# GLAD-RUC/DistEGNN

Measured on NVIDIA H100. Metric: graph_steps_per_sec, higher is better.
Workload: dtype f32

## Files before the change

distegnn_b200/csrc/edge_layer_cs.cu:

```cuda
#include <cuda_fp16.h>
#include <string.h>

#include "common.cuh"
#include "det.cuh"
#include "tc16.cuh"
#include "tile_mma.cuh"

namespace degnn {

struct EdgeCsArgs {
    int64_t N, E;
    const int32_t* E_dev;
    int A;
    unsigned flags;
    const int32_t* row;
    const int32_t* col;
    const float* ea;
    const float* x4;
    const float* P;
    const float* Q;
    const float* w1r;
    const float* w1e;
    const float* w2;
    const float* b2;
    const float* wc;
    const float* bc;
    const float* w3;
    float* agg_m;
    float* agg_x;
    float* slots;
};

constexpr int CS_WG = 4;
constexpr int CS_THREADS = 128 * CS_WG, CS_WARPS = CS_THREADS / 32;
constexpr int CS_TILE = 64;
constexpr int CS_QROW = 72;
constexpr int CS_WBUF = 16 * CS_QROW;
constexpr int CS_IDX = 64;
constexpr int CS_W = 64 * 64;
constexpr int CS_SMEM_BYTES = 4 * CS_W * 2
                              + CS_WARPS * 2 * 8
                              + (4 * H + DISTEGNN_MAX_EDGE_ATTR * H) * 4
                              + CS_WARPS * 2 * CS_WBUF * 4
                              + CS_WARPS * CS_IDX * 4
                              + CS_WARPS * 16 * 8 * 4;
constexpr uint32_t CS_LBO = 1024;

template <int AT, bool LASTL, bool DET>
__global__ void __launch_bounds__(CS_THREADS, 1) edge_layer_cs_kernel(const EdgeCsArgs a) {
    using namespace tmma;
    constexpr int AMAX = AT >= 0 ? (AT > 0 ? AT : 1) : DISTEGNN_MAX_EDGE_ATTR;
    constexpr int AR = (AT == 1 || AT == 2) ? AT : 0;
    constexpr bool need_m = !LASTL;
    __half* W2hi = reinterpret_cast<__half*>(degnn_dyn_smem);
    __half* W2lo = W2hi + CS_W;
    __half* Wchi = W2lo + CS_W;
    __half* Wclo = Wchi + CS_W;
    uint64_t* bars = reinterpret_cast<uint64_t*>(Wclo + CS_W);
    float* b2s = reinterpret_cast<float*>(bars + CS_WARPS * 2);
    float* bcs = b2s + H;
    float* w3s = bcs + H;
    float* w1rs = w3s + H;
    float* w1es = w1rs + H;
    float* qbufs = w1es + DISTEGNN_MAX_EDGE_ATTR * H;
    int* idx_all = reinterpret_cast<int*>(qbufs + CS_WARPS * 2 * CS_WBUF);
    float* xs_all = reinterpret_cast<float*>(idx_all + CS_WARPS * CS_IDX);

    const int tid = threadIdx.x;
    const int lane = tid & 31;
    const int warp = tid >> 5;
    const int wg = warp >> 2;
    const int w = warp & 3;
    const int g = lane >> 2, q = lane & 3;
    const int A = AT >= 0 ? AT : a.A;
    const bool normalize = a.flags & DISTEGNN_FLAG_NORMALIZE;

    tc16::stage_weight<CS_THREADS>(W2hi, W2lo, a.w2, 0, 64, tid, SILU_T_IN);
    tc16::stage_weight<CS_THREADS>(Wchi, Wclo, a.wc, 0, 64, tid);
    if (tid < H) {
        b2s[tid] = a.b2[tid] * SILU_T_IN;
        bcs[tid] = a.bc[tid] * SILU_T_IN;
        w3s[tid] = a.w3[tid] * SILU_T_OUT;
        w1rs[tid] = a.w1r[tid];
    }
    for (int i = tid; i < DISTEGNN_MAX_EDGE_ATTR * H; i += CS_THREADS) w1es[i] = i < A * H ? a.w1e[i] : 0.f;
    for (int i = tid; i < CS_WARPS * 2 * CS_WBUF / 4; i += CS_THREADS)
        reinterpret_cast<float4*>(qbufs)[i] = make_float4(0.f, 0.f, 0.f, 0.f);
    if (tid == 0) {
        for (int i = 0; i < CS_WARPS * 2; ++i) mbar_init(&bars[i], 1);
        fence_mbar_init();
    }
    fence_proxy_async_smem();
    __syncthreads();

    float* qb = qbufs + warp * 2 * CS_WBUF;
    int* nidx = idx_all + warp * CS_IDX;
    float* xs = xs_all + warp * 16 * 8 + 8 * (lane & 15);
    uint64_t* qbar = bars + 2 * warp;
    const uint64_t bW2hi = make_desc(smem_u32(W2hi), CS_LBO, 128), bW2lo = make_desc(smem_u32(W2lo), CS_LBO, 128);
    const uint64_t bWchi = make_desc(smem_u32(Wchi), CS_LBO, 128), bWclo = make_desc(smem_u32(Wclo), CS_LBO, 128);

    const int64_t nE = a.E_dev ? min((int64_t)__ldg(a.E_dev), a.E) : a.E;
    const int64_t num_tiles = (nE + CS_TILE - 1) / CS_TILE;
    const int64_t stride = (int64_t)gridDim.x * CS_WG;
    int64_t tile = (int64_t)blockIdx.x * CS_WG + wg;

    auto edge_of = [&](int64_t tl) { return tl * CS_TILE + 16 * w + lane; };
    auto has_edge = [&](int64_t tl) { return lane < 16 && tl < num_tiles && edge_of(tl) < nE; };
    auto fetch_q = [&](int64_t tl, int b, int col_e, bool v) {
        if (lane == 0) {
            const int64_t nv = min((int64_t)16, max((int64_t)0, nE - (tl * CS_TILE + 16 * w)));
            mbar_expect_tx(qbar + b, (uint32_t)nv * (H * 4));
        }
        if (v) bulk_g2s(qb + b * CS_WBUF + lane * CS_QROW, a.Q + (size_t)col_e * H, H * 4, qbar + b);
    };

    int row_c = -1;
    float dx = 0.f, dy = 0.f, dz = 0.f, radial = 0.f;
    auto set_geometry = [&](float4 xi, float4 xj) {
        dx = xi.x - xj.x; dy = xi.y - xj.y; dz = xi.z - xj.z;
        radial = dx * dx + dy * dy + dz * dz;
        if (normalize) {
            const float inv = 1.0f / (sqrtf(radial) + 1e-8f);
            dx *= inv; dy *= inv; dz *= inv;
        }
    };
    float ea_c[AR > 0 ? AR : 1], n_ea[AR > 0 ? AR : 1];
#pragma unroll
    for (int k = 0; k < (AR > 0 ? AR : 1); ++k) ea_c[k] = n_ea[k] = 0.f;
    int n_row = -1, n_col = 0;

    if (tile < num_tiles) {
        int col_c = 0;
        if (has_edge(tile)) {
            const int64_t e = edge_of(tile);
            row_c = __ldg(a.row + e);
            col_c = __ldg(a.col + e);
#pragma unroll
            for (int k = 0; k < AR; ++k) ea_c[k] = __ldg(a.ea + e * AR + k);
        }
        fetch_q(tile, 0, col_c, row_c >= 0);
        set_geometry(ldg4(a.x4 + (size_t)max(row_c, 0) * 4), ldg4(a.x4 + (size_t)col_c * 4));
        if (has_edge(tile + stride)) {
            const int64_t e = edge_of(tile + stride);
            n_row = __ldg(a.row + e);
            n_col = __ldg(a.col + e);
#pragma unroll
            for (int k = 0; k < AR; ++k) n_ea[k] = __ldg(a.ea + e * AR + k);
        }
    }

    for (int it = 0; tile < num_tiles; ++it, tile += stride) {
        const int64_t ntile = tile + stride, nntile = ntile + stride;
        const int b = it & 1;
        float* qcur = qb + b * CS_WBUF;

        int cont_row = -1;
        if constexpr (DET) {
            const int64_t e0 = tile * CS_TILE + 16 * w;
            const int r0 = __shfl_sync(FULL, row_c, 0);
            if (r0 >= 0 && e0 > 0 && __ldg(a.row + e0 - 1) == r0) cont_row = r0;
        }
        float* const slot = DET ? a.slots + (size_t)(tile * 4 + w) * DET_EDGE_SLOT : nullptr;

        if (ntile < num_tiles) fetch_q(ntile, b ^ 1, n_col, n_row >= 0);
        if (n_row >= 0) {
            cp_async16(xs, a.x4 + (size_t)n_row * 4);
            cp_async16(xs + 4, a.x4 + (size_t)n_col * 4);
            prefetch_l1(a.P + (size_t)n_row * H);
            prefetch_l1(a.P + (size_t)n_row * H + 32);
        }
        if (has_edge(nntile)) {
            const int64_t e = edge_of(nntile);
            cp_async4(nidx + lane, a.row + e);
            cp_async4(nidx + 16 + lane, a.col + e);
            if (AT == 1) cp_async4(nidx + 32 + 2 * lane, a.ea + e);
            if (AT == 2) cp_async8(nidx + 32 + 2 * lane, a.ea + e * 2);
        }
        cp_async_commit();

        const int ra = __shfl_sync(FULL, row_c, g), rb = __shfl_sync(FULL, row_c, g + 8);
        const float rada = __shfl_sync(FULL, radial, g), radb = __shfl_sync(FULL, radial, g + 8);
        float eaa[AMAX], eab[AMAX];
#pragma unroll
        for (int k = 0; k < AMAX; ++k) {
            if (AR > 0) {
                eaa[k] = __shfl_sync(FULL, ea_c[k < AR ? k : 0], g);
                eab[k] = __shfl_sync(FULL, ea_c[k < AR ? k : 0], g + 8);
            } else if (AT < 0) {
                const int64_t e = tile * CS_TILE + 16 * w + g;
                eaa[k] = (k < A && ra >= 0) ? __ldg(a.ea + e * A + k) : 0.f;
                eab[k] = (k < A && rb >= 0) ? __ldg(a.ea + (e + 8) * A + k) : 0.f;
            } else {
                eaa[k] = eab[k] = 0.f;
            }
        }
        const float* pa = a.P + (size_t)max(ra, 0) * H + 2 * q;
        const float* pb = a.P + (size_t)max(rb, 0) * H + 2 * q;
        const float* qa = qcur + g * CS_QROW + 2 * q;
        const float* qbr = qa + 8 * CS_QROW;
        const bool oka = !DET || ra >= 0, okb = !DET || rb >= 0;
        auto pre = [&](int j, const float* prow, const float* qrow, float rad, const float (&ea)[AMAX], bool ok) {
            if (DET && !ok) return bc2(0.f);
            const int c = 8 * j + 2 * q;
            const f32x2 pp = __ldg(reinterpret_cast<const f32x2*>(prow + 8 * j));
            const f32x2 qq = *reinterpret_cast<const f32x2*>(qrow + 8 * j);
            f32x2 p = fma2(bc2(rad), *reinterpret_cast<const f32x2*>(w1rs + c), add2(pp, qq));
#pragma unroll
            for (int k = 0; k < AMAX; ++k)
                if (AT < 0 || k < A)
                    p = fma2(bc2(ea[k]), *reinterpret_cast<const f32x2*>(w1es + k * H + c), p);
            return p;
        };
        uint32_t ahi[16], alo[16];
        float qmax = 0.f;
        auto silu_guard = [&] { return silu_q_overflow(qmax); };
        tc16::RowScales s1;
        mbar_wait(qbar + b, (uint32_t)((it >> 1) & 1));
        tc16::encode_rows<false, true>(
            [&](int j, f32x2& va, f32x2& vb, auto pass) {
                va = pre(j, pa, qa, rada, eaa, oka);
                vb = pre(j, pb, qbr, radb, eab, okb);
                silu4p<decltype(pass)::value != tc16::FAST_PASS>(va, vb, qmax);
            },
            ahi, alo, s1, silu_guard);

        float d[32];
        tc16::mma_f16x3_rA<CS_LBO>(d, ahi, alo, bW2hi, bW2lo);
        const int row_prev = __shfl_up_sync(FULL, row_c, 1);
        const uint32_t M = __ballot_sync(FULL, lane == 0 || row_prev != row_c) & 0xffffu;
        tc16::mma_f16x3_rA_wait(d, ahi, alo);

        qmax = 0.f;
        tc16::RowScales s2;
        tc16::encode_rows<false>(
            [&](int j, f32x2& ma, f32x2& mb, auto pass) {
                const f32x2 bb = *reinterpret_cast<const f32x2*>(b2s + 8 * j + 2 * q);
                ma = fma2(pk2(d[4 * j + 0], d[4 * j + 1]), bc2(s1.inv_a), bb);
                mb = fma2(pk2(d[4 * j + 2], d[4 * j + 3]), bc2(s1.inv_b), bb);
                silu4t<decltype(pass)::value != tc16::FAST_PASS>(ma, mb, qmax);
                if (need_m && decltype(pass)::value != tc16::ENCODE_PASS) {
                    *reinterpret_cast<f32x2*>(qcur + g * CS_QROW + 8 * j + 2 * q) = ma;
                    *reinterpret_cast<f32x2*>(qcur + (g + 8) * CS_QROW + 8 * j + 2 * q) = mb;
                }
            },
            ahi, alo, s2, silu_guard);

        tc16::mma_f16x3_rA<CS_LBO>(d, ahi, alo, bWchi, bWclo);
        if (need_m) {
            __syncwarp();
            const float* colp = qcur + 2 * lane;
            auto flush = [&](f32x2 acc, int e_last) {
                const int rr = __shfl_sync(FULL, row_c, e_last);
                if (rr >= 0) {
                    float v0, v1;
                    upk2(mul2(acc, bc2(SILU_T_OUT)), v0, v1);
                    if constexpr (DET)
                        *reinterpret_cast<float2*>(rr == cont_row ? slot + 2 * lane : a.agg_m + (size_t)rr * H + 2 * lane) =
                            make_float2(v0, v1);
                    else
                        red_add_v2(a.agg_m + (size_t)rr * H + 2 * lane, v0, v1);
                }
            };
            f32x2 s0 = *reinterpret_cast<const f32x2*>(colp);
            if ((M >> 1) == 0u) {
                f32x2 s1 = *reinterpret_cast<const f32x2*>(colp + CS_QROW);
#pragma unroll
                for (int e = 2; e < 16; e += 2) {
                    s0 = add2(s0, *reinterpret_cast<const f32x2*>(colp + e * CS_QROW));
                    s1 = add2(s1, *reinterpret_cast<const f32x2*>(colp + (e + 1) * CS_QROW));
                }
                flush(add2(s0, s1), 15);
            } else {
#pragma unroll
                for (int e = 1; e < 16; ++e) {
                    const f32x2 v = *reinterpret_cast<const f32x2*>(colp + e * CS_QROW);
                    if ((M >> e) & 1u) {
                        flush(s0, e - 1);
                        s0 = v;
                    } else {
                        s0 = add2(s0, v);
                    }
                }
                flush(s0, 15);
            }
        }
        fence_proxy_async_smem();
        __syncwarp();
        tc16::mma_f16x3_rA_wait(d, ahi, alo);

        float phia, phib;
        tc16::phi_head_t(d, s2.inv_a, s2.inv_b, bcs, w3s, q, phia, phib);
        {
            const float fa = __shfl_sync(FULL, phia, 4 * (lane & 7)), fb = __shfl_sync(FULL, phib, 4 * (lane & 7));
            const float phi = (lane & 8) ? fb : fa;
            float sx = dx * phi, sy = dy * phi, sz = dz * phi;
#pragma unroll
            for (int o = 1; o < 16; o <<= 1) {
                const int rk = __shfl_up_sync(FULL, row_c, o);
                const float ox = __shfl_up_sync(FULL, sx, o), oy = __shfl_up_sync(FULL, sy, o), oz = __shfl_up_sync(FULL, sz, o);
                if (lane >= o && rk == row_c) { sx += ox; sy += oy; sz += oz; }
            }
            const int rnext = __shfl_down_sync(FULL, row_c, 1);
            if (row_c >= 0 && (lane == 15 || rnext != row_c)) {
                if constexpr (DET) {
                    float* dst = row_c == cont_row ? slot + H : a.agg_x + (size_t)row_c * 4;
                    dst[0] = sx;
                    dst[1] = sy;
                    dst[2] = sz;
                } else {
                    float* dst = a.agg_x + (size_t)row_c * 4;
                    atomicAdd(dst + 0, sx);
                    atomicAdd(dst + 1, sy);
                    atomicAdd(dst + 2, sz);
                }
            }
        }

        cp_async_wait_all();
        row_c = n_row;
        float4 xi_n = make_float4(0.f, 0.f, 0.f, 0.f), xj_n = xi_n;
        if (n_row >= 0) {
            xi_n = *reinterpret_cast<const float4*>(xs);
            xj_n = *reinterpret_cast<const float4*>(xs + 4);
        }
        set_geometry(xi_n, xj_n);
#pragma unroll
        for (int k = 0; k < AR; ++k) ea_c[k] = n_ea[k];
        n_row = -1;
        if (has_edge(nntile)) {
            n_row = nidx[lane];
            n_col = nidx[16 + lane];
            if (AT == 1) n_ea[0] = __int_as_float(nidx[32 + 2 * lane]);
            if (AT == 2) {
                n_ea[0] = __int_as_float(nidx[32 + 2 * lane]);
                n_ea[AR - 1] = __int_as_float(nidx[33 + 2 * lane]);
            }
        }
    }
}

}

namespace degnn {

template <bool DET>
static int edge_layer_fwd(int64_t n_nodes, int64_t n_edges, int A, int C, int Na, unsigned flags, const int32_t* row,
                          const int32_t* col, const float* edge_attr_sorted, const float* x4, const float* P,
                          const float* Q, const float* layer_params, float* agg_m, float* agg_x,
                          const int32_t* n_edges_dev, void* workspace, int64_t workspace_bytes, void* stream,
                          int max_ctas) {
    if (int rc = check_dims(A, C, Na)) return rc;
    if (n_edges == 0) return DISTEGNN_OK;
    DEGNN_CHECK_ARG(n_nodes > 0 && n_edges > 0, "negative size");
    DEGNN_CHECK_ARG(row && col && x4 && P && Q && layer_params && agg_x, "null pointer");
    DEGNN_CHECK_ARG(A == 0 || edge_attr_sorted, "null edge_attr with edge_attr_nf > 0");
    DEGNN_CHECK_ARG((flags & DISTEGNN_FLAG_LAST) || agg_m, "null agg_m");
    float* slots = nullptr;
    if (DET) {
        if (int rc = det_check_workspace(n_nodes, n_edges, C, workspace, workspace_bytes, "distegnn_edge_layer_fwd_det"))
            return rc;
        slots = det_edge_slots(workspace, n_nodes, C);
    }
    Layout L = make_layout(A, C, Na);
    EdgeCsArgs a;
    a.N = n_nodes; a.E = n_edges; a.E_dev = n_edges_dev; a.A = A; a.flags = flags & 0xffffu;
    a.row = row; a.col = col; a.ea = edge_attr_sorted; a.x4 = x4; a.P = P; a.Q = Q;
    a.w1r = layer_params + L.off[DISTEGNN_P_E_W1R];
    a.w1e = layer_params + L.off[DISTEGNN_P_E_W1E];
    a.w2 = layer_params + L.off[DISTEGNN_P_E_W2];
    a.b2 = layer_params + L.off[DISTEGNN_P_E_B2];
    a.wc = layer_params + L.off[DISTEGNN_P_E_WC];
    a.bc = layer_params + L.off[DISTEGNN_P_E_BC];
    a.w3 = layer_params + L.off[DISTEGNN_P_E_W3];
    a.agg_m = agg_m; a.agg_x = agg_x; a.slots = slots;
    const int64_t tiles = (n_edges + CS_TILE - 1) / CS_TILE;
    int64_t grid = (tiles + CS_WG - 1) / CS_WG;
    if (grid > sm_count()) grid = sm_count();
    if (DET) grid = det_grid(grid, max_ctas);
    auto launch = [&](auto kern) {
        ensure_dynamic_smem((const void*)kern, (int)CS_SMEM_BYTES);
        kern<<<(unsigned)grid, CS_THREADS, CS_SMEM_BYTES, (cudaStream_t)stream>>>(a);
    };
    const bool last = flags & DISTEGNN_FLAG_LAST;
    switch (A) {
        case 0: last ? launch(edge_layer_cs_kernel<0, true, DET>) : launch(edge_layer_cs_kernel<0, false, DET>); break;
        case 1: last ? launch(edge_layer_cs_kernel<1, true, DET>) : launch(edge_layer_cs_kernel<1, false, DET>); break;
        case 2: last ? launch(edge_layer_cs_kernel<2, true, DET>) : launch(edge_layer_cs_kernel<2, false, DET>); break;
        default: last ? launch(edge_layer_cs_kernel<-1, true, DET>) : launch(edge_layer_cs_kernel<-1, false, DET>); break;
    }
    DEGNN_CHECK_LAUNCH();
    return DISTEGNN_OK;
}

int edge_layer_fwd_det(int64_t n_nodes, int64_t n_edges, int A, int C, int Na, unsigned flags, const int32_t* row,
                       const int32_t* col, const float* edge_attr_sorted, const float* x4, const float* P, const float* Q,
                       const float* layer_params, float* agg_m, float* agg_x, const int32_t* n_edges_dev,
                       void* workspace, int64_t workspace_bytes, void* stream, int max_ctas) {
    return edge_layer_fwd<true>(n_nodes, n_edges, A, C, Na, flags, row, col, edge_attr_sorted, x4, P, Q, layer_params,
                                agg_m, agg_x, n_edges_dev, workspace, workspace_bytes, stream, max_ctas);
}

}

extern "C" int distegnn_edge_layer_fwd(int64_t n_nodes, int64_t n_edges, int A, int C, int Na, unsigned flags,
                                       const int32_t* row, const int32_t* col, const float* edge_attr_sorted,
                                       const float* x4, const float* P, const float* Q,
                                       const float* layer_params, float* agg_m, float* agg_x,
                                       const int32_t* n_edges_dev, void* stream) {
    return degnn::edge_layer_fwd<false>(n_nodes, n_edges, A, C, Na, flags, row, col, edge_attr_sorted, x4, P, Q,
                                        layer_params, agg_m, agg_x, n_edges_dev, nullptr, 0, stream, 0);
}

extern "C" int distegnn_edge_layer_fwd_det(int64_t n_nodes, int64_t n_edges, int A, int C, int Na, unsigned flags,
                                           const int32_t* row, const int32_t* col, const float* edge_attr_sorted,
                                           const float* x4, const float* P, const float* Q,
                                           const float* layer_params, float* agg_m, float* agg_x,
                                           const int32_t* n_edges_dev, void* workspace, int64_t workspace_bytes,
                                           void* stream) {
    return degnn::edge_layer_fwd_det(n_nodes, n_edges, A, C, Na, flags, row, col, edge_attr_sorted, x4, P, Q,
                                     layer_params, agg_m, agg_x, n_edges_dev, workspace, workspace_bytes, stream, 0);
}
```

distegnn_b200/csrc/tile_mma.cuh:

```cuda
#pragma once
#include <cuda_runtime.h>
#include <stdint.h>

namespace degnn {

extern __shared__ __align__(1024) uint8_t degnn_dyn_smem[];

namespace tmma {

constexpr uint32_t TM_COLGROUP_BYTES = 2048;
__host__ __device__ constexpr int tm_bytes(int ncols) { return ncols * 128 * 4; }

__device__ __forceinline__ uint32_t smem_u32(const void* p) {
    return (uint32_t)__cvta_generic_to_shared(p);
}

__device__ __forceinline__ uint32_t tm_addr_rc(uint32_t row, uint32_t col) {
    return smem_u32(degnn_dyn_smem) + (col >> 2) * TM_COLGROUP_BYTES + row * 16u + (col & 3u) * 4u;
}
__device__ __forceinline__ uint32_t tm_addr(uint32_t taddr) {
    return tm_addr_rc((taddr >> 16) + (threadIdx.x & 31u), taddr & 0xffffu);
}

__device__ __forceinline__ uint64_t make_desc(uint32_t smem_addr, uint32_t lbo, uint32_t sbo) {
    return (uint64_t)((smem_addr >> 4) & 0x3FFF) | ((uint64_t)((lbo >> 4) & 0x3FFF) << 16) |
           ((uint64_t)((sbo >> 4) & 0x3FFF) << 32);
}

__device__ __forceinline__ void fence_proxy_async_smem() { asm volatile("fence.proxy.async.shared::cta;" ::: "memory"); }

__device__ __forceinline__ void tm_st4(uint32_t taddr, const uint32_t (&r)[4]) {
    asm volatile("st.shared.v4.b32 [%0], {%1,%2,%3,%4};" ::"r"(tm_addr(taddr)), "r"(r[0]), "r"(r[1]), "r"(r[2]), "r"(r[3])
                 : "memory");
}
__device__ __forceinline__ void tm_ld4(uint32_t taddr, uint32_t* r) {
    asm volatile("ld.shared.v4.b32 {%0,%1,%2,%3}, [%4];" : "=r"(r[0]), "=r"(r[1]), "=r"(r[2]), "=r"(r[3]) : "r"(tm_addr(taddr))
                 : "memory");
}
__device__ __forceinline__ void tm_st8(uint32_t taddr, const uint32_t (&r)[8]) {
    tm_st4(taddr, *reinterpret_cast<const uint32_t(*)[4]>(&r[0]));
    tm_st4(taddr + 4, *reinterpret_cast<const uint32_t(*)[4]>(&r[4]));
}
__device__ __forceinline__ void tm_st16(uint32_t taddr, const uint32_t (&r)[16]) {
#pragma unroll
    for (int i = 0; i < 4; ++i) tm_st4(taddr + 4 * i, *reinterpret_cast<const uint32_t(*)[4]>(&r[4 * i]));
}
__device__ __forceinline__ void tm_ld16(uint32_t taddr, uint32_t (&r)[16]) {
#pragma unroll
    for (int i = 0; i < 4; ++i) tm_ld4(taddr + 4 * i, &r[4 * i]);
}
__device__ __forceinline__ void prefetch_l1(const void* p) { asm volatile("prefetch.global.L1 [%0];" ::"l"(p)); }
__device__ __forceinline__ void prefetch_l2(const void* p) { asm volatile("prefetch.global.L2 [%0];" ::"l"(p)); }

__device__ __forceinline__ void wgmma_fence() { asm volatile("wgmma.fence.sync.aligned;" ::: "memory"); }
__device__ __forceinline__ void wgmma_commit() { asm volatile("wgmma.commit_group.sync.aligned;" ::: "memory"); }
__device__ __forceinline__ void wgmma_wait_all() { asm volatile("wgmma.wait_group.sync.aligned 0;" ::: "memory"); }
__device__ __forceinline__ void wgmma_f16_m64n64k16(float (&d)[32], uint64_t a_desc, uint64_t b_desc, uint32_t accumulate) {
    asm volatile(
        "{\n\t"
        ".reg .pred p;\n\t"
        "setp.ne.b32 p, %34, 0;\n\t"
        "wgmma.mma_async.sync.aligned.m64n64k16.f32.f16.f16 "
        "{%0,%1,%2,%3,%4,%5,%6,%7,%8,%9,%10,%11,%12,%13,%14,%15,%16,%17,%18,%19,%20,%21,%22,%23,%24,%25,%26,%27,%28,%29,%30,%31},"
        " %32, %33, p, 1, 1, 0, 0;\n\t"
        "}\n"
        : "+f"(d[0]), "+f"(d[1]), "+f"(d[2]), "+f"(d[3]), "+f"(d[4]), "+f"(d[5]), "+f"(d[6]), "+f"(d[7]), "+f"(d[8]),
          "+f"(d[9]), "+f"(d[10]), "+f"(d[11]), "+f"(d[12]), "+f"(d[13]), "+f"(d[14]), "+f"(d[15]), "+f"(d[16]),
          "+f"(d[17]), "+f"(d[18]), "+f"(d[19]), "+f"(d[20]), "+f"(d[21]), "+f"(d[22]), "+f"(d[23]), "+f"(d[24]),
          "+f"(d[25]), "+f"(d[26]), "+f"(d[27]), "+f"(d[28]), "+f"(d[29]), "+f"(d[30]), "+f"(d[31])
        : "l"(a_desc), "l"(b_desc), "r"(accumulate)
        : "memory");
}
#define DEGNN_WGMMA_RA_D(c)                                                                                             \
    c(d[0]), c(d[1]), c(d[2]), c(d[3]), c(d[4]), c(d[5]), c(d[6]), c(d[7]), c(d[8]), c(d[9]), c(d[10]), c(d[11]),      \
        c(d[12]), c(d[13]), c(d[14]), c(d[15]), c(d[16]), c(d[17]), c(d[18]), c(d[19]), c(d[20]), c(d[21]), c(d[22]),  \
        c(d[23]), c(d[24]), c(d[25]), c(d[26]), c(d[27]), c(d[28]), c(d[29]), c(d[30]), c(d[31])
#define DEGNN_WGMMA_RA_ASM(scale_d)                                                                                     \
    "wgmma.mma_async.sync.aligned.m64n64k16.f32.f16.f16 "                                                               \
    "{%0,%1,%2,%3,%4,%5,%6,%7,%8,%9,%10,%11,%12,%13,%14,%15,%16,%17,%18,%19,%20,%21,%22,%23,%24,%25,%26,%27,%28,%29,%30," \
    "%31}, {%32,%33,%34,%35}, %36, " scale_d ", 1, 1, 0;\n"
template <bool ACCUMULATE>
__device__ __forceinline__ void wgmma_f16_m64n64k16_rA(float (&d)[32], uint32_t a0, uint32_t a1, uint32_t a2, uint32_t a3,
                                                       uint64_t b_desc) {
    if (ACCUMULATE)
        asm volatile(DEGNN_WGMMA_RA_ASM("1") : DEGNN_WGMMA_RA_D("+f")
                     : "r"(a0), "r"(a1), "r"(a2), "r"(a3), "l"(b_desc) : "memory");
    else
        asm volatile(DEGNN_WGMMA_RA_ASM("0") : DEGNN_WGMMA_RA_D("=f")
                     : "r"(a0), "r"(a1), "r"(a2), "r"(a3), "l"(b_desc) : "memory");
}
#undef DEGNN_WGMMA_RA_D
#undef DEGNN_WGMMA_RA_ASM
__device__ __forceinline__ void wgmma_keep(float& r) { asm volatile("" : "+f"(r)::"memory"); }
__device__ __forceinline__ void wgmma_keep(uint32_t& r) { asm volatile("" : "+r"(r)::"memory"); }
__device__ __forceinline__ void frag_rows(int mb, uint32_t& r0, uint32_t& q) {
    const uint32_t w = (threadIdx.x >> 5) & 3u, l = threadIdx.x & 31u;
    r0 = 64u * (uint32_t)mb + 16u * w + (l >> 2);
    q = l & 3u;
}
__device__ __forceinline__ void frag_store(const float (&d)[32], uint32_t col, int mb) {
    uint32_t r0, q;
    frag_rows(mb, r0, q);
#pragma unroll
    for (int j = 0; j < 8; ++j) {
        const uint32_t c = col + 8u * j + 2u * q;
        const uint32_t a0 = tm_addr_rc(r0, c), a1 = tm_addr_rc(r0 + 8u, c);
        asm volatile("st.shared.v2.f32 [%0], {%1,%2};" ::"r"(a0), "f"(d[4 * j]), "f"(d[4 * j + 1]) : "memory");
        asm volatile("st.shared.v2.f32 [%0], {%1,%2};" ::"r"(a1), "f"(d[4 * j + 2]), "f"(d[4 * j + 3]) : "memory");
    }
}
__device__ __forceinline__ void frag_load(float (&d)[32], uint32_t col, int mb) {
    uint32_t r0, q;
    frag_rows(mb, r0, q);
#pragma unroll
    for (int j = 0; j < 8; ++j) {
        const uint32_t c = col + 8u * j + 2u * q;
        asm volatile("ld.shared.v2.f32 {%0,%1}, [%2];" : "=f"(d[4 * j]), "=f"(d[4 * j + 1]) : "r"(tm_addr_rc(r0, c)) : "memory");
        asm volatile("ld.shared.v2.f32 {%0,%1}, [%2];" : "=f"(d[4 * j + 2]), "=f"(d[4 * j + 3]) : "r"(tm_addr_rc(r0 + 8u, c))
                     : "memory");
    }
}

__device__ __forceinline__ void mbar_init(uint64_t* bar, uint32_t count) {
    asm volatile("mbarrier.init.shared::cta.b64 [%0], %1;" ::"r"(smem_u32(bar)), "r"(count) : "memory");
}
__device__ __forceinline__ void fence_mbar_init() { asm volatile("fence.mbarrier_init.release.cluster;" ::: "memory"); }
__device__ __forceinline__ void mbar_expect_tx(uint64_t* bar, uint32_t bytes) {
    asm volatile("mbarrier.arrive.expect_tx.shared::cta.b64 _, [%0], %1;" ::"r"(smem_u32(bar)), "r"(bytes) : "memory");
}
__device__ __forceinline__ void mbar_wait(uint64_t* bar, uint32_t parity) {
    asm volatile(
        "{\n\t"
        ".reg .pred p;\n\t"
        "WAIT_LOOP:\n\t"
        "mbarrier.try_wait.parity.shared::cta.b64 p, [%0], %1;\n\t"
        "@p bra WAIT_DONE;\n\t"
        "bra WAIT_LOOP;\n\t"
        "WAIT_DONE:\n\t"
        "}\n" ::"r"(smem_u32(bar)),
        "r"(parity)
        : "memory");
}

__device__ __forceinline__ void bulk_g2s(void* smem_dst, const void* gsrc, uint32_t bytes, uint64_t* bar) {
    asm volatile("cp.async.bulk.shared::cluster.global.mbarrier::complete_tx::bytes [%0], [%1], %2, [%3];" ::"r"(
                     smem_u32(smem_dst)),
                 "l"(gsrc), "r"(bytes), "r"(smem_u32(bar))
                 : "memory");
}

__device__ __forceinline__ void cp_async16(void* smem_dst, const void* gsrc) {
    asm volatile("cp.async.cg.shared.global [%0], [%1], 16;" ::"r"(smem_u32(smem_dst)), "l"(gsrc) : "memory");
}
__device__ __forceinline__ void cp_async8(void* smem_dst, const void* gsrc) {
    asm volatile("cp.async.ca.shared.global [%0], [%1], 8;" ::"r"(smem_u32(smem_dst)), "l"(gsrc) : "memory");
}
__device__ __forceinline__ void cp_async4(void* smem_dst, const void* gsrc) {
    asm volatile("cp.async.ca.shared.global [%0], [%1], 4;" ::"r"(smem_u32(smem_dst)), "l"(gsrc) : "memory");
}
__device__ __forceinline__ void cp_async_commit() { asm volatile("cp.async.commit_group;" ::: "memory"); }
__device__ __forceinline__ void cp_async_wait_all() { asm volatile("cp.async.wait_group 0;" ::: "memory"); }
__device__ __forceinline__ void red_add_v2(float* gdst, float a, float b) {
    asm volatile("red.global.add.v2.f32 [%0], {%1, %2};" ::"l"(gdst), "f"(a), "f"(b) : "memory");
}

__device__ __forceinline__ void named_bar(uint32_t id, uint32_t nthreads) {
    asm volatile("bar.sync %0, %1;" ::"r"(id), "r"(nthreads) : "memory");
}

}
}
```

Before: 36.47.

## Replace per-row bulk TMA Q gather with warp-cooperative cp.async and 32-bit indexing

Q rows for each tile's column nodes are now gathered with warp-cooperative 16-byte cp.async copies instead of per-lane cp.async.bulk transfers tracked by mbarriers. The mbarrier setup, waits and async-proxy fences are removed, and completion is handled by the existing cp.async wait group plus a syncwarp. Edge, tile and stride indices move from 64-bit to 32-bit arithmetic, with hoisted base pointers, to cut address math. A host check now rejects edge counts near 2^31.

Measured after the change: 37.70 (median of 6 runs). 3.4% higher.

```diff
diff --git a/distegnn_b200/csrc/edge_layer_cs.cu b/distegnn_b200/csrc/edge_layer_cs.cu
--- a/distegnn_b200/csrc/edge_layer_cs.cu
+++ b/distegnn_b200/csrc/edge_layer_cs.cu
@@ -9,7 +9,8 @@
 namespace degnn {
 
 struct EdgeCsArgs {
-    int64_t N, E;
+    int64_t N;
+    int E;
     const int32_t* E_dev;
     int A;
     unsigned flags;
@@ -39,7 +40,6 @@
 constexpr int CS_IDX = 64;
 constexpr int CS_W = 64 * 64;
 constexpr int CS_SMEM_BYTES = 4 * CS_W * 2
-                              + CS_WARPS * 2 * 8
                               + (4 * H + DISTEGNN_MAX_EDGE_ATTR * H) * 4
                               + CS_WARPS * 2 * CS_WBUF * 4
                               + CS_WARPS * CS_IDX * 4
@@ -56,8 +56,7 @@
     __half* W2lo = W2hi + CS_W;
     __half* Wchi = W2lo + CS_W;
     __half* Wclo = Wchi + CS_W;
-    uint64_t* bars = reinterpret_cast<uint64_t*>(Wclo + CS_W);
-    float* b2s = reinterpret_cast<float*>(bars + CS_WARPS * 2);
+    float* b2s = reinterpret_cast<float*>(Wclo + CS_W);
     float* bcs = b2s + H;
     float* w3s = bcs + H;
     float* w1rs = w3s + H;
@@ -86,33 +85,34 @@
     for (int i = tid; i < DISTEGNN_MAX_EDGE_ATTR * H; i += CS_THREADS) w1es[i] = i < A * H ? a.w1e[i] : 0.f;
     for (int i = tid; i < CS_WARPS * 2 * CS_WBUF / 4; i += CS_THREADS)
         reinterpret_cast<float4*>(qbufs)[i] = make_float4(0.f, 0.f, 0.f, 0.f);
-    if (tid == 0) {
-        for (int i = 0; i < CS_WARPS * 2; ++i) mbar_init(&bars[i], 1);
-        fence_mbar_init();
-    }
     fence_proxy_async_smem();
     __syncthreads();
 
     float* qb = qbufs + warp * 2 * CS_WBUF;
     int* nidx = idx_all + warp * CS_IDX;
     float* xs = xs_all + warp * 16 * 8 + 8 * (lane & 15);
-    uint64_t* qbar = bars + 2 * warp;
+    const float* Pq = a.P + 2 * q;
+    asm("" : "+l"(Pq));
     const uint64_t bW2hi = make_desc(smem_u32(W2hi), CS_LBO, 128), bW2lo = make_desc(smem_u32(W2lo), CS_LBO, 128);
     const uint64_t bWchi = make_desc(smem_u32(Wchi), CS_LBO, 128), bWclo = make_desc(smem_u32(Wclo), CS_LBO, 128);
 
-    const int64_t nE = a.E_dev ? min((int64_t)__ldg(a.E_dev), a.E) : a.E;
-    const int64_t num_tiles = (nE + CS_TILE - 1) / CS_TILE;
-    const int64_t stride = (int64_t)gridDim.x * CS_WG;
-    int64_t tile = (int64_t)blockIdx.x * CS_WG + wg;
-
-    auto edge_of = [&](int64_t tl) { return tl * CS_TILE + 16 * w + lane; };
-    auto has_edge = [&](int64_t tl) { return lane < 16 && tl < num_tiles && edge_of(tl) < nE; };
-    auto fetch_q = [&](int64_t tl, int b, int col_e, bool v) {
-        if (lane == 0) {
-            const int64_t nv = min((int64_t)16, max((int64_t)0, nE - (tl * CS_TILE + 16 * w)));
-            mbar_expect_tx(qbar + b, (uint32_t)nv * (H * 4));
-        }
-        if (v) bulk_g2s(qb + b * CS_WBUF + lane * CS_QROW, a.Q + (size_t)col_e * H, H * 4, qbar + b);
+    const int nE = a.E_dev ? min(__ldg(a.E_dev), a.E) : a.E;
+    const int num_tiles = (nE + CS_TILE - 1) / CS_TILE;
+    const int stride = gridDim.x * CS_WG;
+    int tile = blockIdx.x * CS_WG + wg;
+
+    auto edge_of = [&](int tl) { return tl * CS_TILE + 16 * w + lane; };
+    auto has_edge = [&](int tl) { return lane < 16 && tl < num_tiles && edge_of(tl) < nE; };
+    auto fetch_q = [&](int b, int col_e) {
+        const int cols = __shfl_sync(FULL, col_e, (lane & 15) + (lane >> 4));
+        const uint32_t dst = smem_u32(qb + b * CS_WBUF + (lane >> 4) * CS_QROW + 4 * (lane & 15));
+        const char* src = reinterpret_cast<const char*>(a.Q + 4 * (lane & 15));
+        asm("" : "+l"(src));
+#pragma unroll
+        for (int k = 0; k < 8; ++k) {
+            const int c = __shfl_sync(FULL, cols, 2 * k, 16);
+            if (c >= 0) cp_async16(dst + 2 * k * CS_QROW * 4, src + (size_t)(uint32_t)c * (H * 4));
+        }
     };
 
     int row_c = -1;
@@ -133,37 +133,40 @@
     if (tile < num_tiles) {
         int col_c = 0;
         if (has_edge(tile)) {
-            const int64_t e = edge_of(tile);
+            const int e = edge_of(tile);
             row_c = __ldg(a.row + e);
             col_c = __ldg(a.col + e);
 #pragma unroll
-            for (int k = 0; k < AR; ++k) ea_c[k] = __ldg(a.ea + e * AR + k);
-        }
-        fetch_q(tile, 0, col_c, row_c >= 0);
+            for (int k = 0; k < AR; ++k) ea_c[k] = __ldg(a.ea + (size_t)e * AR + k);
+        }
+        fetch_q(0, row_c >= 0 ? col_c : -1);
+        cp_async_commit();
         set_geometry(ldg4(a.x4 + (size_t)max(row_c, 0) * 4), ldg4(a.x4 + (size_t)col_c * 4));
         if (has_edge(tile + stride)) {
-            const int64_t e = edge_of(tile + stride);
+            const int e = edge_of(tile + stride);
             n_row = __ldg(a.row + e);
             n_col = __ldg(a.col + e);
 #pragma unroll
-            for (int k = 0; k < AR; ++k) n_ea[k] = __ldg(a.ea + e * AR + k);
-        }
+            for (int k = 0; k < AR; ++k) n_ea[k] = __ldg(a.ea + (size_t)e * AR + k);
+        }
+        cp_async_wait_all();
+        __syncwarp();
     }
 
     for (int it = 0; tile < num_tiles; ++it, tile += stride) {
-        const int64_t ntile = tile + stride, nntile = ntile + stride;
+        const int nntile = tile + 2 * stride;
         const int b = it & 1;
         float* qcur = qb + b * CS_WBUF;
 
         int cont_row = -1;
         if constexpr (DET) {
-            const int64_t e0 = tile * CS_TILE + 16 * w;
+            const int e0 = tile * CS_TILE + 16 * w;
             const int r0 = __shfl_sync(FULL, row_c, 0);
             if (r0 >= 0 && e0 > 0 && __ldg(a.row + e0 - 1) == r0) cont_row = r0;
         }
         float* const slot = DET ? a.slots + (size_t)(tile * 4 + w) * DET_EDGE_SLOT : nullptr;
 
-        if (ntile < num_tiles) fetch_q(ntile, b ^ 1, n_col, n_row >= 0);
+        fetch_q(b ^ 1, n_row >= 0 ? n_col : -1);
         if (n_row >= 0) {
             cp_async16(xs, a.x4 + (size_t)n_row * 4);
             cp_async16(xs + 4, a.x4 + (size_t)n_col * 4);
@@ -171,11 +174,11 @@
             prefetch_l1(a.P + (size_t)n_row * H + 32);
         }
         if (has_edge(nntile)) {
-            const int64_t e = edge_of(nntile);
+            const int e = edge_of(nntile);
             cp_async4(nidx + lane, a.row + e);
             cp_async4(nidx + 16 + lane, a.col + e);
             if (AT == 1) cp_async4(nidx + 32 + 2 * lane, a.ea + e);
-            if (AT == 2) cp_async8(nidx + 32 + 2 * lane, a.ea + e * 2);
+            if (AT == 2) cp_async8(nidx + 32 + 2 * lane, a.ea + (size_t)e * 2);
         }
         cp_async_commit();
 
@@ -188,15 +191,15 @@
                 eaa[k] = __shfl_sync(FULL, ea_c[k < AR ? k : 0], g);
                 eab[k] = __shfl_sync(FULL, ea_c[k < AR ? k : 0], g + 8);
             } else if (AT < 0) {
-                const int64_t e = tile * CS_TILE + 16 * w + g;
-                eaa[k] = (k < A && ra >= 0) ? __ldg(a.ea + e * A + k) : 0.f;
-                eab[k] = (k < A && rb >= 0) ? __ldg(a.ea + (e + 8) * A + k) : 0.f;
+                const int e = tile * CS_TILE + 16 * w + g;
+                eaa[k] = (k < A && ra >= 0) ? __ldg(a.ea + (size_t)e * A + k) : 0.f;
+                eab[k] = (k < A && rb >= 0) ? __ldg(a.ea + (size_t)(e + 8) * A + k) : 0.f;
             } else {
                 eaa[k] = eab[k] = 0.f;
             }
         }
-        const float* pa = a.P + (size_t)max(ra, 0) * H + 2 * q;
-        const float* pb = a.P + (size_t)max(rb, 0) * H + 2 * q;
+        const float* pa = Pq + (size_t)(uint32_t)max(ra, 0) * H;
+        const float* pb = Pq + (size_t)(uint32_t)max(rb, 0) * H;
         const float* qa = qcur + g * CS_QROW + 2 * q;
         const float* qbr = qa + 8 * CS_QROW;
         const bool oka = !DET || ra >= 0, okb = !DET || rb >= 0;
@@ -216,7 +219,6 @@
         float qmax = 0.f;
         auto silu_guard = [&] { return silu_q_overflow(qmax); };
         tc16::RowScales s1;
-        mbar_wait(qbar + b, (uint32_t)((it >> 1) & 1));
         tc16::encode_rows<false, true>(
             [&](int j, f32x2& va, f32x2& vb, auto pass) {
                 va = pre(j, pa, qa, rada, eaa, oka);
@@ -250,16 +252,18 @@
         if (need_m) {
             __syncwarp();
             const float* colp = qcur + 2 * lane;
+            float* mrow = a.agg_m + 2 * lane;
+            asm("" : "+l"(mrow));
             auto flush = [&](f32x2 acc, int e_last) {
                 const int rr = __shfl_sync(FULL, row_c, e_last);
                 if (rr >= 0) {
                     float v0, v1;
                     upk2(mul2(acc, bc2(SILU_T_OUT)), v0, v1);
                     if constexpr (DET)
-                        *reinterpret_cast<float2*>(rr == cont_row ? slot + 2 * lane : a.agg_m + (size_t)rr * H + 2 * lane) =
+                        *reinterpret_cast<float2*>(rr == cont_row ? slot + 2 * lane : mrow + (size_t)(uint32_t)rr * H) =
                             make_float2(v0, v1);
                     else
-                        red_add_v2(a.agg_m + (size_t)rr * H + 2 * lane, v0, v1);
+                        red_add_v2(mrow + (size_t)(uint32_t)rr * H, v0, v1);
                 }
             };
             f32x2 s0 = *reinterpret_cast<const f32x2*>(colp);
@@ -285,8 +289,6 @@
                 flush(s0, 15);
             }
         }
-        fence_proxy_async_smem();
-        __syncwarp();
         tc16::mma_f16x3_rA_wait(d, ahi, alo);
 
         float phia, phib;
@@ -318,6 +320,7 @@
         }
 
         cp_async_wait_all();
+        __syncwarp();
         row_c = n_row;
         float4 xi_n = make_float4(0.f, 0.f, 0.f, 0.f), xj_n = xi_n;
         if (n_row >= 0) {
@@ -353,6 +356,7 @@
     if (int rc = check_dims(A, C, Na)) return rc;
     if (n_edges == 0) return DISTEGNN_OK;
     DEGNN_CHECK_ARG(n_nodes > 0 && n_edges > 0, "negative size");
+    DEGNN_CHECK_ARG(n_edges <= INT32_MAX - (CS_TILE - 1), "n_edges (the capacity with n_edges_dev) above 2^31 - 64");
     DEGNN_CHECK_ARG(row && col && x4 && P && Q && layer_params && agg_x, "null pointer");
     DEGNN_CHECK_ARG(A == 0 || edge_attr_sorted, "null edge_attr with edge_attr_nf > 0");
     DEGNN_CHECK_ARG((flags & DISTEGNN_FLAG_LAST) || agg_m, "null agg_m");
@@ -364,7 +368,7 @@
     }
     Layout L = make_layout(A, C, Na);
     EdgeCsArgs a;
-    a.N = n_nodes; a.E = n_edges; a.E_dev = n_edges_dev; a.A = A; a.flags = flags & 0xffffu;
+    a.N = n_nodes; a.E = (int)n_edges; a.E_dev = n_edges_dev; a.A = A; a.flags = flags & 0xffffu;
     a.row = row; a.col = col; a.ea = edge_attr_sorted; a.x4 = x4; a.P = P; a.Q = Q;
     a.w1r = layer_params + L.off[DISTEGNN_P_E_W1R];
     a.w1e = layer_params + L.off[DISTEGNN_P_E_W1E];
diff --git a/distegnn_b200/csrc/tile_mma.cuh b/distegnn_b200/csrc/tile_mma.cuh
--- a/distegnn_b200/csrc/tile_mma.cuh
+++ b/distegnn_b200/csrc/tile_mma.cuh
@@ -149,9 +149,10 @@
                  : "memory");
 }
 
-__device__ __forceinline__ void cp_async16(void* smem_dst, const void* gsrc) {
-    asm volatile("cp.async.cg.shared.global [%0], [%1], 16;" ::"r"(smem_u32(smem_dst)), "l"(gsrc) : "memory");
+__device__ __forceinline__ void cp_async16(uint32_t smem_addr, const void* gsrc) {
+    asm volatile("cp.async.cg.shared.global [%0], [%1], 16;" ::"r"(smem_addr), "l"(gsrc) : "memory");
 }
+__device__ __forceinline__ void cp_async16(void* smem_dst, const void* gsrc) { cp_async16(smem_u32(smem_dst), gsrc); }
 __device__ __forceinline__ void cp_async8(void* smem_dst, const void* gsrc) {
     asm volatile("cp.async.ca.shared.global [%0], [%1], 8;" ::"r"(smem_u32(smem_dst)), "l"(gsrc) : "memory");
 }
```
